# rubendhz/houdini-gsplat-renderer

Hardware: AMD Instinct MI355X
Metric: frames/sec at 1920x1080 + achieved HBM GB/s (blend kernel) (higher is better)
Workload: dtype f32

## Files before the change

houdini-gsplat-renderer_amd/csrc/gsr_api.hip:

```cpp
#include <hip/hip_runtime.h>

#include <cmath>
#include <cstdarg>
#include <cstdio>
#include <cstring>
#include <chrono>
#include <algorithm>
#include <new>
#include <vector>

#include "../../include/gsplat_hip.h"
#include "gsr_device.h"
#include "k_binning.h"
#include "k_blend.h"
#include "k_cluster.h"
#include "k_colour.h"
#include "k_preprocess.h"
#ifdef GSR_HOST_TIMING
static double g_t_verdict = 0, g_acc_py = 0, g_acc_pre = 0, g_acc_launch = 0; static long g_acc_n = 0;
static double now_us() { return std::chrono::duration<double, std::micro>(std::chrono::steady_clock::now().time_since_epoch()).count(); }
#endif
#include "k_sort.h"
#include "k_wire.h"
#include "gsr_frame_plan.h"
// ... 105 lines not shown
    float* dpyr = nullptr;
    size_t dpyr_cap = 0;
    uint32_t* dactive = nullptr;
    int dpar = 0;
    bool dpyr_built = false;
    bool sorted_dculled = false;
    uint32_t* hist = nullptr;
    size_t hist_cap = 0;
    uint32_t* totals = nullptr;
    uint2* pvA = nullptr;
    size_t pair_cap = 0;
    int32_t *sstart = nullptr, *send = nullptr;
    uint4* tile_work = nullptr;
    size_t tile_cap = 0;
    uint4* tile_work_a = nullptr;
    float* tbuf = nullptr;
    size_t tbuf_cap = 0;
    float* hpyr2 = nullptr;
    uint32_t* slab = nullptr;
    bool slab_dirty = false;
    int32_t* redo = nullptr;
    int32_t* order = nullptr;
    size_t order_cap = 0;
    bool order_valid = false;
    int order_age = 0;
    int order_sig[6] = {0, 0, 0, 0, 0, 0}, order_per_xcd = 0;
    uint32_t* st_scan = nullptr;
    GsrTilePartial* partial = nullptr;
    uint32_t* sup_work = nullptr;
    int sup_par = 0;
// ... 268 lines not shown
    return ok;
}

static void slot_free_splat_arrays(FrameSlot& sl)
{
    dev_free(sl.rec); dev_free(sl.keyA); dev_free(sl.keyB); dev_free(sl.valA); dev_free(sl.valB); dev_free(sl.blk_cnt);
    dev_free(sl.zwin); dev_free(sl.cseg);
    sl.sort_valid = false;
}

static void slot_destroy(FrameSlot& sl)
{
    slot_free_splat_arrays(sl);
    dev_free(sl.hist); dev_free(sl.totals);
    dev_free(sl.pvA);
    dev_free(sl.sstart); dev_free(sl.send); dev_free(sl.tile_work); dev_free(sl.order); dev_free(sl.sup_work); dev_free(sl.fb); dev_free(sl.fb32); dev_free(sl.aovb); dev_free(sl.bgb);
    dev_free(sl.hpyr); dev_free(sl.hpyr_next); dev_free(sl.hraw); dev_free(sl.hstat); dev_free(sl.hpyr2); dev_free(sl.slab); dev_free(sl.tile_work_a); dev_free(sl.tbuf); dev_free(sl.ccnt); dev_free(sl.bkt_key); dev_free(sl.bkt_val); dev_free(sl.bkt_cnt); dev_free(sl.d_counts); dev_free(sl.st_scan); dev_free(sl.partial);
    if (sl.h_end) (void)hipHostFree(sl.h_end); dev_free(sl.depth_stage); dev_free(sl.dpyr); dev_free(sl.dactive);
    dev_free(sl.redo); dev_free(sl.lazy_ctr); dev_free(sl.colour_evals);
    dev_free(sl.counters); dev_free(sl.d_n);
    if (sl.h_total) (void)hipHostFree(sl.h_total);
    if (sl.h_counters) (void)hipHostFree(sl.h_counters);
    dev_free(sl.d_frame);
    if (sl.ev_ok)
        for (int k = 0; k < GSR_STAGE_EVENTS; ++k)
            if (sl.ev[k]) (void)hipEventDestroy(sl.ev[k]);
    if (sl.ev_done) (void)hipEventDestroy(sl.ev_done);
    if (sl.ev_user) (void)hipEventDestroy(sl.ev_user);
    for (int k = 0; k < GSR_HOST_BANDS_MAX; ++k) if (sl.ev_band[k]) (void)hipEventDestroy(sl.ev_band[k]);
    if (sl.ev_pairs) (void)hipEventDestroy(sl.ev_pairs);
    if (sl.own) (void)hipStreamDestroy(sl.own);
// ... 820 lines not shown
    if (j.timing && (j.timing_all || k >= 5)) HIP_TRY(hipEventRecord(sl.ev[k], sl.stream));
    return GSR_OK;
}

static GsrRangeArgs range_args(gsr_context* c, FrameSlot& sl)
{
    const FrameJob& j = sl.job;
    GsrRangeArgs a;
    a.totals = sl.totals; a.n_super = j.n_super; a.sstart = sl.sstart; a.send = sl.send; a.host_total = sl.h_total_dev;
    a.ticket = j.ticket; a.max_pairs = (unsigned long long)GSR_MAX_PAIRS; a.redo_count = reinterpret_cast<uint32_t*>(sl.lazy_ctr);
    a.lazy_hint = c->lazy_hint; a.n_sorted = sl.d_n; a.k1_counts = sl.d_counts; a.sorted_keys = sl.keyA;
    a.depth_active = j.dcull ? sl.dactive + j.dpar : (const uint32_t*)nullptr;
    return a;
}

static int queue_blend(gsr_context* c, FrameSlot& sl, bool with_depth, bool guarded)
{
    const FrameJob& j = sl.job;
    const GsrFrame& f = j.f;
    hipStream_t s = sl.stream;
    if (j.local_tiles > 0) {
        if (!j.direct) HIP_TRY(hipStreamWaitEvent(s, sl.ev_user, 0));
        GsrBlendArgs a;
        a.guard = guarded ? sl.dactive + j.dpar : (const uint32_t*)nullptr; a.guard_want = 0u;
        {
            const bool persp = f.pr[8] == 0.0f && f.pr[9] == 0.0f && f.pr[12] == 0.0f && f.pr[13] == 0.0f && f.pr[14] == -1.0f && f.pr[15] == 0.0f;
            a.near_alpha = persp ? 0.5f * (1.0f - f.pr[10]) : 0.0f;
            a.near_scale = persp ? 1.12f : 0.0f;
        }
        a.tile_cov = (with_depth && j.dcull && !j.dblind) ? sl.dpyr + 4 * sl.dpyr_cap : (const float*)nullptr;
        a.idx_mask = f.idx_mask; a.zq0 = f.zq0; a.zqs = f.zqs;
        a.tile_dmax = (with_depth && j.dcull && !j.dblind && f.idx_mask != 0xffffffffu) ? sl.dpyr + (size_t)(2 * j.dpar) * sl.dpyr_cap + f.pyr_off[0] : (const float*)nullptr;
        a.width = f.width; a.height = f.height; a.tiles_x = f.tiles_x; a.local_tiles = j.local_tiles;
        a.shard = GsrShard{f.shard_index, f.shard_count, f.shard_rpb}; a.band_rows = j.band_rows;
        a.super_shift = f.super_shift; a.rect_shift = f.rect_shift; a.stiles_x = f.stiles_x; a.use_map = j.use_map ? 1 : 0; a.flags = f.flags;
        a.list_cap = (int32_t)std::min<size_t>(sl.pair_cap, (size_t)0x7fffffff);
        a.sup_work = (a.use_map && c->opt_swizzle >= 2 && sl.sup_work) ? sl.sup_work + 256 * sl.sup_par : nullptr;
        a.slab = j.phase; a.tbuf = sl.tbuf; a.tile_work_a = sl.tile_work_a;
// ... 98 lines not shown
        HIP_TRY(hipGetLastError());
    }
    if ((rc = mark(sl, 5))) return rc;
    sl.job.blend_guess_plain = j.d_depth != nullptr && j.dcull && !c->depth_active && !j.deferred && j.f.idx_mask == 0xffffffffu && !j.aov_target && j.bg.kind == 0;
    if ((rc = queue_blend(c, sl, j.d_depth != nullptr && !sl.job.blend_guess_plain, sl.job.blend_guess_plain))) return rc;
    return mark(sl, 6);
}

static int queue_frame_end(gsr_context* c, FrameSlot& sl)
{
    const FrameJob& j = sl.job;
    hipStream_t s = sl.stream;
    GsrSumArgs g;
    g.n_tiles = j.local_tiles; g.tiles_x = j.f.tiles_x; g.tiles_y = j.f.tiles_y; g.shard = GsrShard{j.f.shard_index, j.f.shard_count, j.f.shard_rpb};
    g.super_shift = j.f.super_shift; g.stiles_x = j.f.stiles_x; g.n_super = j.n_super;
    GsrHorizonArgs hz{};
    hz.list_cap = (int32_t)std::min<size_t>(sl.pair_cap, (size_t)0x7fffffff);
    if (c->opt_cull && c->opt_cull != 3 && j.n > 0 && !j.deferred && (c->opt_cull >= 2 || j.cull || j.phase == 2 || (c->cull_pol.vis_unculled >= 300000u && c->cull_pol.holdoff <= 2))) {
        hz.raw = sl.hraw; hz.pyr_in = sl.hpyr; hz.pyr_out = sl.hpyr_next; hz.dilate = j.f.cull_dilate; hz.culled = j.cull ? 1 : 0; hz.lists = sl.pvA; hz.geoA = c->geoA;
        for (int l = 0; l < GSR_PYR_LEVELS; ++l) hz.pyr_off[l] = j.f.pyr_off[l];
        hz.cam[0] = j.f.cam[0]; hz.cam[1] = j.f.cam[1]; hz.cam[2] = j.f.cam[2];
        hz.host_end = j.cull ? sl.h_end_dev : nullptr; hz.ticket = j.ticket;
        hz.stat = sl.hstat;
        hz.stat_in_use = (j.cull && j.dcull && j.dstat) ? 1 : 0;
        hz.depth_culled = (j.dcull && !j.dblind) ? 1 : 0;
        hz.idx_mask = j.f.idx_mask;
        static const bool dbgv = std::getenv("GSR_DEBUG_VIOL") != nullptr;
        if (dbgv) {
            if (!sl.dbg_viol && hipMalloc(reinterpret_cast<void**>(&sl.dbg_viol), 80 * 4) != hipSuccess) sl.dbg_viol = nullptr;
            if (sl.dbg_viol) (void)hipMemsetAsync(sl.dbg_viol, 0, 80 * 4, s);
            hz.dbg = sl.dbg_viol;
        }
    }
    if (j.phase == 2) { hz.slab = 2; hz.tile_work_a = sl.tile_work_a; }
    const int nblocks8 = ((j.f.tiles_x + 7) >> 3) * ((j.f.tiles_y + 7) >> 3);
    hipLaunchKernelGGL(k_tile_pass, dim3((unsigned)nblocks8), dim3(64), 0, s, sl.tile_work, g, sl.sstart, sl.send, hz, sl.partial, sl.st_scan);
    uint32_t* const prefix_arg = (j.f.sh_order > 0 && c->opt_lazy) ? c->prefix : (uint32_t*)nullptr;
    const uint32_t* const redo_arg = j.lazy ? reinterpret_cast<const uint32_t*>(sl.lazy_ctr) : (const uint32_t*)nullptr;
    uint32_t* const work_next = sl.sup_work ? sl.sup_work + 256 * (sl.sup_par ^ 1) : (uint32_t*)nullptr;
    sl.horizon_valid = hz.raw != nullptr;
    sl.hstat_valid = hz.raw != nullptr;
    const int osig[6] = {j.f.width, j.f.height, j.f.shard_index, j.f.shard_count, j.f.shard_rpb, j.f.super_shift};
    const bool order_due = c->opt_swizzle >= 3 || (c->opt_swizzle == 2 && c->order_pays);
    const bool order_kept = !order_due && c->opt_swizzle == 2 && c->opt_order_keep > 0 && sl.order_valid && sl.order_age < c->opt_order_keep &&
                            std::memcmp(osig, sl.order_sig, sizeof osig) == 0;
    const bool order_refresh = !order_due && !order_kept && c->opt_swizzle == 2 && c->opt_order_keep > 0 && c->n >= 1000000u;
    if (order_kept) sl.order_age += 1; else sl.order_valid = false;
    const bool order_now = j.use_map && (order_due || order_refresh) && j.local_tiles > 0 && j.n_super <= 256 && sl.sup_work;
    const int per_xcd = 2 * ((j.n_super + 15) / 16) << (2 * j.f.super_shift);
    if (order_now) {
        const size_t want = (size_t)8 * per_xcd;
        if (want > sl.order_cap) {
            HIP_TRY(hipStreamSynchronize(s));
            dev_free(sl.order);
            sl.order_cap = 0;
            int rc = dev_alloc(&sl.order, want);
            if (rc) return rc;
            sl.order_cap = want;
        }
    }
    const bool fused_order = order_now && c->opt_fuse_order != 0;
    if (sl.horizon_valid) sl.hpyr_re = std::min(c->cull_pol.dilate, GSR_DILATE_EXACT_MAX);
    if (fused_order) {
        const GsrOrderArgs oa{sl.tile_work, j.f.tiles_y, sl.sup_work + 256 * sl.sup_par, per_xcd, sl.order};
        const int ndil = sl.horizon_valid ? nblocks8 : 0;
        hipLaunchKernelGGL(k_frame_end_order, dim3(9u + (unsigned)((ndil + TO_THREADS / 64 - 1) / (TO_THREADS / 64))), dim3(TO_THREADS), 0, s, sl.partial, nblocks8, ndil, g, sl.counters, sl.d_n, sl.d_frame,
                           prefix_arg, redo_arg, sl.colour_evals, sl.lazy_ctr + 1, sl.sstart, sl.send, c->lazy_hint, work_next, hz, sl.st_scan, sl.hpyr_re, oa);
        HIP_TRY(hipGetLastError());
    } else if (sl.horizon_valid) {
        hipLaunchKernelGGL(k_frame_end, dim3((unsigned)nblocks8 + 1u), dim3(SW_THREADS), 0, s, sl.partial, nblocks8, g, sl.counters, sl.d_n, sl.d_frame,
                           prefix_arg, redo_arg, sl.colour_evals, sl.lazy_ctr + 1, sl.sstart, sl.send, c->lazy_hint, work_next, hz, sl.st_scan, sl.hpyr_re);
        HIP_TRY(hipGetLastError());
    } else {
        hipLaunchKernelGGL(k_sum_work, dim3(1), dim3(SW_THREADS), 0, s, sl.partial, nblocks8, g, sl.counters, sl.d_n, sl.d_frame,
                           prefix_arg, redo_arg, sl.colour_evals, sl.lazy_ctr + 1, sl.sstart, sl.send, c->lazy_hint, work_next, hz, sl.st_scan);
        HIP_TRY(hipGetLastError());
    }
    if (sl.horizon_valid) {
        std::swap(sl.hpyr, sl.hpyr_next);
        const int sig[7] = {j.f.width, j.f.height, j.f.shard_index, j.f.shard_count, j.f.shard_rpb, j.f.super_shift, (int)c->geo_gen};
        std::memcpy(sl.horizon_sig, sig, sizeof sig);
        sl.horizon_cam = j.args.cam;
    }
    if (order_now) {
        if (!fused_order) {
            hipLaunchKernelGGL(k_tile_order, dim3(8), dim3(TO_THREADS), 0, s, sl.tile_work, g, j.f.tiles_y, sl.sup_work + 256 * sl.sup_par,
                               per_xcd, sl.order);
            HIP_TRY(hipGetLastError());
        }
        std::memcpy(sl.order_sig, osig, sizeof osig);
// ... 115 lines not shown
template <typename T>
static int regrow(hipStream_t s, T*& p, size_t& cap, size_t count, size_t new_cap)
{
    HIP_TRY(hipStreamSynchronize(s));
    dev_free(p);
    cap = 0;
    const int rc = dev_alloc(&p, count);
    if (rc) return rc;
    cap = new_cap;
    return GSR_OK;
}

static int abandon_attempt(FrameSlot& sl, bool redo)
{
    if (sl.sup_work) (void)hipMemsetAsync(sl.sup_work + 256 * sl.sup_par, 0, 256 * sizeof(uint32_t), sl.stream);
    sl.sort_valid = false;
    sl.job.redo = redo;
    sl.job.open = false;
    return GSR_OK;
}

static int render_again(gsr_context* c, const FrameArgs& a, int phase, FrameSlot** used)
{
    c->frame_no -= 1;
    c->st.frames -= 1;
    FrameSlot* sl = nullptr;
    int rc = frame_begin(c, a, &sl, false, phase);
    if (rc) return rc;
    if ((rc = frame_finish(c, *sl))) return rc;
    if (used) *used = sl;
// ... 51 lines not shown
    if (o.grow) {
        const size_t floor_ = sl.pvA ? 0 : std::min<size_t>((size_t)2 * j.n + 4096, (size_t)1 << 22);
        const size_t want = std::max<size_t>((size_t)D + D / 4 + 4096, std::max(floor_, c->pair_want));
        const int rc = regrow(sl.stream, sl.pvA, sl.pair_cap, want + 4, want);
        if (rc) return frame_abort(sl, rc);
        c->pair_want = std::max(c->pair_want, want);
    }
    if (o.end == GSR_FE_SLAB_OVERRUN) {
        c->st.frames_requeued += 1;
        return abandon_attempt(sl, true);
    }
    if (o.back_end == GSR_BE_TRUNCATED) c->st.frames_truncated += 1;
    if (o.back_end == GSR_BE_REQUEUED) {
        c->st.frames_requeued += 1;
        if (sl.sup_work) (void)hipMemsetAsync(sl.sup_work + 256 * sl.sup_par, 0, 256 * sizeof(uint32_t), sl.stream);
    }
    if (o.back_end == GSR_BE_QUEUED || o.back_end == GSR_BE_REQUEUED) {
        const int rc = queue_back_end(c, sl);
        if (rc) return frame_abort(sl, rc);
    }
    sl.last_pairs = D;
    if (o.guard_miss) {
        j.blend_guess_plain = false;
        const int rc = queue_blend(c, sl, true, false);
        if (rc) return frame_abort(sl, rc);
    }
    if (o.end == GSR_FE_PHASE_2) {
        const int rc = queue_slab_mid(c, sl);
        if (rc) return frame_abort(sl, rc);
        if (j.timing) { sl.ev_pending = true; sl.ev_all = false; }
// ... 120 lines not shown
    j.dcull = p.dcull; j.local_sort = p.local || p.local_phase; j.bn_items = p.bn_items; j.bn_grid = p.bn_grid; j.k1_grid = p.k1_grid;
    j.f.cull_dilate = p.cull_dilate;
    j.f.phase = p.phase;
    c->st.frames_jumped += p.jumped;
    c->st.frames_culled += p.cull;
    c->st.frames_slab += p.phase == 1;
    c->st.frames_lazy += p.lazy && n > 0 && phase_in == 0;
    j.ticket = ++sl.ticket ? sl.ticket : ++sl.ticket;
    if (j.timing) harvest_slot(c, sl);

    j.direct = sl.stream == c->stream;
    if (!j.direct) HIP_TRY(hipEventRecord(sl.ev_user, c->stream));

    if ((size_t)j.local_tiles + 1 > sl.tile_cap || !sl.sstart) {
        HIP_TRY(hipStreamSynchronize(s));
        dev_free(sl.tile_work); dev_free(sl.tile_work_a); dev_free(sl.sstart); dev_free(sl.send); dev_free(sl.redo);
        sl.tile_cap = 0;
        if ((rc = dev_alloc(&sl.tile_work, (size_t)j.local_tiles + 1)) || (rc = dev_alloc(&sl.tile_work_a, (size_t)j.local_tiles + 1)) || (rc = dev_alloc(&sl.sstart, (size_t)65536 + 1)) ||
            (rc = dev_alloc(&sl.send, (size_t)65536 + 1)) || (rc = dev_alloc(&sl.redo, (size_t)j.local_tiles + 1))) return rc;
        sl.tile_cap = (size_t)j.local_tiles + 1;
    }
    if (j.phase == 1 && j.out_px > sl.tbuf_cap && (rc = regrow(s, sl.tbuf, sl.tbuf_cap, j.out_px, j.out_px))) return rc;
    if (j.use_map && (rc = build_tile_map(c, f))) return rc;
    j.d_depth = a.depth;
    if (a.depth && !a.depth_is_device) {
        const size_t npx = (size_t)cam->width * cam->height;
        if (npx > sl.depth_cap && (rc = regrow(s, sl.depth_stage, sl.depth_cap, npx, npx))) return rc;
        HIP_TRY(hipMemcpyAsync(sl.depth_stage, a.depth, npx * 4, hipMemcpyHostToDevice, s));
        j.d_depth = sl.depth_stage;
    }
    if (a.bg.kind != 0) {
        j.bg.kind = a.bg.kind; j.bg.format = a.bg.format;
        std::memcpy(j.bg.rgba, a.bg.rgba, sizeof j.bg.rgba);
// ... 820 lines not shown
```

houdini-gsplat-renderer_amd/csrc/gsr_device.h:

```cpp
#pragma once
#ifdef GSR_KPROF
#include <hip/hip_runtime.h>
__device__ unsigned long long g_kprof[8][16];
__device__ unsigned int g_kprof_blk[5][2][8192];
#define KPROF_BLK_BEGIN const unsigned long long kp0_ = wall_clock64();
#define KPROF_BLK_END(k, items) { if (threadIdx.x == 0 && blockIdx.x < 8192) { g_kprof_blk[k][0][blockIdx.x] = (unsigned int)(wall_clock64() - kp0_); g_kprof_blk[k][1][blockIdx.x] = (unsigned int)(items); } }
#define KPROF(k, i) { if (blockIdx.x == 0 && threadIdx.x == 0) g_kprof[k][i] = wall_clock64(); }
#define KPROFB(k, i, blk) { if (blockIdx.x == (blk) && threadIdx.x == 0) g_kprof[k][i] = wall_clock64(); }
#else
#define KPROF(k, i)
#define KPROFB(k, i, blk)
#define KPROF_BLK_BEGIN
#define KPROF_BLK_END(k, items)
#endif

#include <hip/hip_runtime.h>
#include <stdint.h>
#include "gsr_mailbox.h"

#define GSR_TILE_PX 16
#define GSR_WAVE 64

struct __attribute__((aligned(16))) GsrRecord {
    float cx, cy, hx, hy;
// ... 33 lines not shown
    int32_t rect_shift;
    int32_t phase;
    uint32_t idx_mask;
    float zq0, zqs;
};
#define GSR_ZQ_SHIFT 23
#define GSR_ZQ_MAX 511.0f
#define GSR_SLAB_BINS 1024
#define GSR_FLAG_NO_ALPHA_RADIUS 1
#define GSR_FLAG_NO_SAT          2
#define GSR_FLAG_FULL_KEYS       4
#define GSR_FLAG_LAZY_NO_PREFIX  8
#define GSR_FLAG_CULL_ROUNDS    16
#define GSR_FLAG_NO_DEPTH_CLASS 32
#define GSR_FLAG_NO_ZCODES      64

#ifndef BK_BUCKETS
#define BK_BUCKETS 1024
#endif
#ifndef BK_CAP
#define BK_CAP 8192
#endif
#define BK_STRIDE 64

__device__ __forceinline__ float gsr_fma(float a, float b, float c) { return __builtin_fmaf(a, b, c); }

__device__ __forceinline__ uint32_t gsr_zq(float zw, float z0, float zs)
{
    const float t = __builtin_fminf(__builtin_fmaxf((zw - z0) * zs, 0.0f), GSR_ZQ_MAX);
    return (uint32_t)t;
// ... 185 lines not shown
```

houdini-gsplat-renderer_amd/csrc/k_blend.h:

```cpp
#pragma once
#include <type_traits>
#include "gsr_device.h"
#include "k_preprocess.h"
#include "k_cluster.h"

#ifndef BL_ROUND
#define BL_ROUND 64
#endif
#ifndef BL_WAVES_PER_EU
#define BL_WAVES_PER_EU 6
#endif
#ifndef BL_CHECK
#define BL_CHECK 4
#endif
#ifndef BL_BATCH
#define BL_BATCH 256
#endif
#ifndef BL_CHECK_AOVD
#define BL_CHECK_AOVD 2
#endif
#define BL_QCAP 2048
#define BL_PAIR_F4_MAX 6
#define GSR_T_MIN 6.103515625e-05f

#ifdef BL_PROFILE
#define BLP_MAX_WG 65536
__device__ unsigned long long g_blend_prof[BLP_MAX_WG][4][16];
#define BLP(i) { const long long now_ = clock64(); prof[i] += (unsigned long long)(now_ - tlast); tlast = now_; }
#else
#define BLP(i)
#endif

__device__ __forceinline__ uint32_t gsr_tile_weight(const uint4& w) { return w.z * 32u + w.y * 8u + (w.x >> 1); }

#ifdef GSR_DEBUG_XCC
__device__ uint32_t g_dbg_xcc[4];
#endif
struct GsrBlendArgs {
    int32_t width, height;
    int32_t tiles_x;
    int32_t local_tiles;
    GsrShard shard;
    int32_t band_rows;
    int32_t super_shift;
    int32_t rect_shift;
    int32_t stiles_x;
    int32_t use_map;
    int32_t flags;
    int32_t list_cap;
    uint32_t* sup_work;
    int32_t slab;
    float* tbuf;
    const uint4* tile_work_a;
    const uint32_t* guard;
    uint32_t guard_want;
    float near_alpha, near_scale;
    const float* tile_cov;
    uint32_t idx_mask;
    float zq0, zqs;
    const float* tile_dmax;
    int32_t row_lo, row_hi;
    int32_t out_format;
    void* out_packed;
};

#if BL_WAVES_PER_EU > 0
#define BL_OCC __attribute__((amdgpu_waves_per_eu(BL_WAVES_PER_EU)))
#else
#define BL_OCC
#endif
struct GsrLazyArgs {
    GsrFrame f;
    const uint4* colrow;
    int32_t* redo;
    uint32_t* redo_count;
};
struct GsrBgArgs {
    int32_t kind;
    int32_t format;
    float rgba[4];
    const void* image;
};
template <bool HAS_DEPTH, bool LAZY, bool AOV = false, bool OVER = false>
__device__ __forceinline__ void
gsr_blend_tile(const GsrBlendArgs& a, const int32_t* __restrict__ tile_map, const uint2* __restrict__ svals,
               const int32_t* __restrict__ sstart, const int32_t* __restrict__ send,
               const GsrRecord* __restrict__ recs, float4* __restrict__ out, uint4* __restrict__ tile_work,
               const float* __restrict__ zwin, const float* __restrict__ depth, const GsrLazyArgs& lz, float2* __restrict__ aov = nullptr,
               const GsrBgArgs* __restrict__ bg = nullptr)
{
    constexpr bool ZSTAGE = HAS_DEPTH || AOV;
    constexpr int PF4 = 5;
    __shared__ float4 slist[4][(BL_ROUND / 2) * PF4];
    __shared__ float2 szl[ZSTAGE ? 4 : 1][ZSTAGE ? BL_ROUND / 2 : 1];
    __shared__ uint32_t q[BL_QCAP];
    __shared__ __attribute__((aligned(16))) uint32_t scnt[2][4];
    __shared__ uint32_t sdone[2][4];
// ... 49 lines not shown

    const int st = (gty >> a.super_shift) * a.stiles_x + (tx >> a.super_shift);
    const int s = sstart[st];
    const int e_ = send[st] < a.list_cap ? send[st] : a.list_cap;
    const int n = e_ > s ? e_ - s : 0;
    if (!HAS_DEPTH && a.guard && (guard_now != 0u) != (a.guard_want != 0u)) return;

    gsr_v2f C01 = {0.0f, 0.0f};
    float C2 = 0.0f, T = 1.0f;
    float Z = 0.0f;
    bool wave_done = false;
    if (a.slab == 2) {
        const uint4 wa = a.tile_work_a[tile];
        if (wa.w & 1u) {
            if (tid == 0) tile_work[tile] = make_uint4(0u, 0u, 0u, 1u | 0x8000u | (0xffffu << 16));
            return;
        }
        if (pix_ok) {
            const size_t at = (size_t)(lty * GSR_TILE_PX + (wave >> 1) * 8 + (lane >> 3)) * a.width + (size_t)(tx * GSR_TILE_PX + (wave & 1) * 8 + (lane & 7));
            const float4 c = out[at];
            C01 = (gsr_v2f){c.x, c.y}; C2 = c.z; T = a.tbuf[at];
            if constexpr (AOV) Z = aov[at].x;
        }
        wave_done = __all(!pix_ok || T < GSR_T_MIN);
    }
    bool u_done = false;
    uint32_t my_last_u = 0;
    uint32_t es_u = 0xffu;
    bool u_all = false;
    uint32_t fetched = 0;
// ... 322 lines not shown
        for (int i = 0; i < 9; ++i) o[i] = prof[i];
        o[9] = 1ull; o[10] = (unsigned long long)round; o[11] = wall0; o[12] = wall_clock64();
        o[13] = occ_lanes; o[14] = occ_evals; o[15] = occ_half | (occ_none << 32);
    }
#endif
    __syncthreads();
    if (lane == 0) { atomicAdd(&sevals, my_evals); if (HAS_DEPTH && d_met) sdmet = 1u; }
    __syncthreads();
    if (HAS_DEPTH && !d_init) init_depth();
    const uint32_t es_c = ext_steps_of(max(max(slast[0], slast[1]), max(slast[2], slast[3])));
    if (!HAS_DEPTH) { u_all = saturated; es_u = es_c; }
    else if (!u_all) {
        const uint32_t dl = sdone[(round - 1) & 1][0] & sdone[(round - 1) & 1][1] & sdone[(round - 1) & 1][2] & sdone[(round - 1) & 1][3];
        if (round > 0 ? (dl & 2u) != 0u : __syncthreads_and(u_done ? 1 : 0) != 0) { u_all = true; es_u = round > 0 ? ext_steps_of(max(max(slastu[0], slastu[1]), max(slastu[2], slastu[3]))) : 0u; }
    }
    if (tid == 0) {
        const int rd = scan_pos + 1024;
        const uint32_t fs = (uint32_t)(first_hit_step < 0 ? 0 : (first_hit_step > 0x1fff ? 0x1fff : first_hit_step)) | (sdmet ? 0x2000u : 0u);
        const uint4 tw = make_uint4((uint32_t)(rd < n ? rd : n), fetched, sevals, (saturated ? 1u : 0u) | (fs << 1) | (u_all ? 0x8000u : 0u) | (es_c << 16) | (es_u << 24));
        tile_work[tile] = tw;
        if (a.sup_work && gsr_tile_weight(tw)) atomicAdd(&a.sup_work[st], gsr_tile_weight(tw));
    }
}

template <bool HAS_DEPTH>
__global__ void __launch_bounds__(256) BL_OCC
k_blend(GsrBlendArgs a, const int32_t* __restrict__ tile_map, const uint2* __restrict__ svals,
        const int32_t* __restrict__ sstart, const int32_t* __restrict__ send,
        const GsrRecord* __restrict__ recs, float4* __restrict__ out, uint4* __restrict__ tile_work,
        const float* __restrict__ zwin, const float* __restrict__ depth, GsrLazyArgs lz)
{
    gsr_blend_tile<HAS_DEPTH, false>(a, tile_map, svals, sstart, send, recs, out, tile_work, zwin, depth, lz);
}
template <bool HAS_DEPTH>
__global__ void __launch_bounds__(256)
k_blend_lazy(GsrBlendArgs a, const int32_t* __restrict__ tile_map, const uint2* __restrict__ svals,
             const int32_t* __restrict__ sstart, const int32_t* __restrict__ send,
// ... 253 lines not shown
        if (own) h = !opaque ? __builtin_inff() : (c2 ? hnew : slab_d2 * 1.05f);
        if (inside) hz.raw[gty * g.tiles_x + tx] = (own && !(opaque && (w.w & 0x4000u) == 0u)) ? -h : h;
    }
}

__device__ __forceinline__ void
gsr_sum_work(const GsrTilePartial* __restrict__ partial, int nblocks, GsrSumArgs g, unsigned long long* __restrict__ counters,
           const uint32_t* __restrict__ n_visible, unsigned long long* __restrict__ summary ,
           uint32_t* __restrict__ prefix ,
           const uint32_t* __restrict__ redo_count ,
           uint32_t* __restrict__ colour_evals ,
           unsigned long long* __restrict__ colour_total ,
           const int32_t* __restrict__ sstart, const int32_t* __restrict__ send,
           uint32_t* __restrict__ lazy_hint ,
           uint32_t* __restrict__ sup_work_next ,
           GsrHorizonArgs hz, uint32_t* __restrict__ st_scan )
{
    SWP(0)
    __shared__ unsigned long long s_sum[3];
    __shared__ uint32_t s_unsat, s_est, s_cev, s_wmax, s_nfin, s_nused, s_viol;
    unsigned long long old2 = 0, old4 = 0, old5 = 0, old_ct = 0;
    uint32_t nvis = 0, nredo = 0, my_cev = 0, my_m = 0;
    int my_s0 = 0, my_e0 = 0;
    if (threadIdx.x == 0) {
        old2 = counters[2]; old4 = counters[4]; old5 = counters[5];
        nvis = *n_visible;
        nredo = redo_count ? *redo_count : 0u;
        if (colour_evals) old_ct = *colour_total;
        s_unsat = 0; s_est = 0; s_cev = 0; s_wmax = 0; s_nfin = 0; s_nused = 0; s_viol = 0;
    }
    if (threadIdx.x < 3) s_sum[threadIdx.x] = 0;
    if (colour_evals) my_cev = colour_evals[threadIdx.x];
    if ((int)threadIdx.x < g.n_super) { my_m = st_scan[threadIdx.x]; my_s0 = sstart[threadIdx.x]; my_e0 = send[threadIdx.x]; }
    unsigned long long sc = 0, fe = 0, ev = 0;
    uint32_t wmax = 0, unsat = 0, nused = 0, nfin = 0, viol = 0;
    for (int i = (int)threadIdx.x; i < nblocks; i += SW_THREADS) {
        const GsrTilePartial p = partial[i];
        sc += p.scanned; fe += p.fetched; ev += p.evals; unsat += p.unsat; nused += p.nused; nfin += p.nfin; viol |= p.viol;
        wmax = p.wmax > wmax ? p.wmax : wmax;
    }
    __syncthreads();
#pragma unroll
    for (int d = 32; d > 0; d >>= 1) {
        sc += __shfl_down(sc, d, 64); fe += __shfl_down(fe, d, 64); ev += __shfl_down(ev, d, 64); unsat += __shfl_down(unsat, d, 64);
        nused += __shfl_down(nused, d, 64); nfin += __shfl_down(nfin, d, 64);
        { const uint32_t o = __shfl_down(wmax, d, 64); wmax = o > wmax ? o : wmax; }
    }
    const bool any_viol = __ballot(viol != 0u) != 0ull;
    if ((threadIdx.x & 63) == 0) {
        atomicAdd(&s_sum[0], sc); atomicAdd(&s_sum[1], fe); atomicAdd(&s_sum[2], ev); atomicAdd(&s_unsat, unsat); atomicMax(&s_wmax, wmax);
// ... 35 lines not shown
                                    ((hz.culled || ((unsigned long long)s_nfin * 10ull >= (unsigned long long)s_nused * 3ull && s_nused > 0u)) ? GSR_HINT_CULL_PAYS : 0u);
        const unsigned long long t2 = old2 + s_sum[1], t4 = old4 + s_sum[0], t5 = old5 + s_sum[2];
        counters[1] = s_sum[1]; counters[2] = t2; counters[3] = s_sum[0]; counters[4] = t4; counters[5] = t5;
        if (colour_evals) *colour_total = old_ct + s_cev;
        summary[0] = 0ull; summary[1] = s_sum[1]; summary[2] = t2; summary[3] = s_sum[0]; summary[4] = t4; summary[5] = t5;
        summary[6] = (unsigned long long)nvis;
        summary[7] = (unsigned long long)nredo;
    }
    SWP(5)
}
__global__ void __launch_bounds__(SW_THREADS)
k_sum_work(const GsrTilePartial* __restrict__ partial, int nblocks, GsrSumArgs g, unsigned long long* __restrict__ counters,
           const uint32_t* __restrict__ n_visible, unsigned long long* __restrict__ summary, uint32_t* __restrict__ prefix,
           const uint32_t* __restrict__ redo_count, uint32_t* __restrict__ colour_evals, unsigned long long* __restrict__ colour_total,
           const int32_t* __restrict__ sstart, const int32_t* __restrict__ send, uint32_t* __restrict__ lazy_hint,
           uint32_t* __restrict__ sup_work_next, GsrHorizonArgs hz, uint32_t* __restrict__ st_scan)
{
    gsr_sum_work(partial, nblocks, g, counters, n_visible, summary, prefix, redo_count, colour_evals, colour_total, sstart, send, lazy_hint,
                 sup_work_next, hz, st_scan);
}

__device__ __forceinline__ void
gsr_horizon_dilate(const float* __restrict__ raw, int tiles_x, int tiles_y, int r, const GsrHorizonArgs& hz, float* __restrict__ pyr, const int b,
                   const int lane )
{
    const int lx = (lane & 1) | ((lane >> 1) & 2) | ((lane >> 2) & 4), ly = ((lane >> 1) & 1) | ((lane >> 2) & 2) | ((lane >> 3) & 4);
    const int nbx = (tiles_x + 7) >> 3;
    const int by = b / nbx, bx = b - by * nbx;
    const int tx = bx * 8 + lx, ty = by * 8 + ly;
    const bool inside = tx < tiles_x && ty < tiles_y;
    float v = 0.0f;
    if (inside) {
        const int x0 = max(tx - r, 0), x1 = min(tx + r, tiles_x - 1), y0 = max(ty - r, 0), y1 = min(ty + r, tiles_y - 1);
        bool allc = true;
// ... 16 lines not shown
        atomicMax(reinterpret_cast<uint32_t*>(pyr) + hz.pyr_off[4] + (by >> 1) * gsr_pyr_dim(tiles_x, 4) + (bx >> 1), __float_as_uint(v));
        atomicMax(reinterpret_cast<uint32_t*>(pyr) + hz.pyr_off[5] + (by >> 2) * gsr_pyr_dim(tiles_x, 5) + (bx >> 2), __float_as_uint(v));
    }
}
__global__ void __launch_bounds__(64)
k_horizon_dilate(const float* __restrict__ raw, int tiles_x, int tiles_y, int r, GsrHorizonArgs hz, float* __restrict__ pyr)
{
    gsr_horizon_dilate(raw, tiles_x, tiles_y, r, hz, pyr, (int)blockIdx.x, (int)threadIdx.x);
}

__global__ void __launch_bounds__(SW_THREADS)
k_frame_end(const GsrTilePartial* __restrict__ partial, int nblocks, GsrSumArgs g, unsigned long long* __restrict__ counters,
            const uint32_t* __restrict__ n_visible, unsigned long long* __restrict__ summary, uint32_t* __restrict__ prefix,
            const uint32_t* __restrict__ redo_count, uint32_t* __restrict__ colour_evals, unsigned long long* __restrict__ colour_total,
            const int32_t* __restrict__ sstart, const int32_t* __restrict__ send, uint32_t* __restrict__ lazy_hint,
            uint32_t* __restrict__ sup_work_next, GsrHorizonArgs hz, uint32_t* __restrict__ st_scan, int dilate_r)
{
    if ((int)blockIdx.x == nblocks) {
        gsr_sum_work(partial, nblocks, g, counters, n_visible, summary, prefix, redo_count, colour_evals, colour_total, sstart, send, lazy_hint,
                     sup_work_next, hz, st_scan);
        return;
    }
    if (threadIdx.x >= 64) return;
    gsr_horizon_dilate(hz.raw, g.tiles_x, g.tiles_y, dilate_r, hz, hz.pyr_out, (int)blockIdx.x, (int)threadIdx.x);
}

#define TO_THREADS 1024
#define TO_LEVELS 128
__device__ __forceinline__ void
gsr_tile_order(const uint4* __restrict__ tile_work, const GsrSumArgs& g, int tiles_y, const uint32_t* __restrict__ sup_work, int cap,
               int32_t* __restrict__ order, const int xcd)
{
    __shared__ uint32_t s_sup[256];
    __shared__ uint32_t s_own[64];
    __shared__ uint32_t s_hist[TO_LEVELS];
// ... 84 lines not shown
}
__global__ void __launch_bounds__(TO_THREADS)
k_tile_order(const uint4* __restrict__ tile_work, GsrSumArgs g, int tiles_y, const uint32_t* __restrict__ sup_work, int cap,
             int32_t* __restrict__ order)
{
    gsr_tile_order(tile_work, g, tiles_y, sup_work, cap, order, (int)blockIdx.x);
}

struct GsrOrderArgs { const uint4* tile_work; int32_t tiles_y; const uint32_t* sup_work; int32_t cap; int32_t* order; };
__global__ void __launch_bounds__(TO_THREADS)
k_frame_end_order(const GsrTilePartial* __restrict__ partial, int nblocks, int ndilate , GsrSumArgs g,
                  unsigned long long* __restrict__ counters, const uint32_t* __restrict__ n_visible, unsigned long long* __restrict__ summary,
                  uint32_t* __restrict__ prefix, const uint32_t* __restrict__ redo_count, uint32_t* __restrict__ colour_evals,
                  unsigned long long* __restrict__ colour_total, const int32_t* __restrict__ sstart, const int32_t* __restrict__ send,
                  uint32_t* __restrict__ lazy_hint, uint32_t* __restrict__ sup_work_next, GsrHorizonArgs hz, uint32_t* __restrict__ st_scan, int dilate_r,
                  GsrOrderArgs oa)
{
    const int b = (int)blockIdx.x;
    if (b < 8) {
        gsr_tile_order(oa.tile_work, g, oa.tiles_y, oa.sup_work, oa.cap, oa.order, b);
        return;
    }
    if (b == 8) {
        if (threadIdx.x >= SW_THREADS) return;
        gsr_sum_work(partial, nblocks, g, counters, n_visible, summary, prefix, redo_count, colour_evals, colour_total, sstart, send, lazy_hint,
                     sup_work_next, hz, st_scan);
        return;
    }
    static_assert(TO_THREADS % 64 == 0 && SW_THREADS % 64 == 0, "early exits are by whole wavefronts");
    const int blk = (b - 9) * (TO_THREADS / 64) + (int)(threadIdx.x >> 6);
    if (blk >= ndilate) return;
    gsr_horizon_dilate(hz.raw, g.tiles_x, g.tiles_y, dilate_r, hz, hz.pyr_out, blk, (int)(threadIdx.x & 63u));
}
```

Measured before the change: 4433.

## Fold tile-pass horizon/stat work into blend kernel epilogue

Moves the per-tile post-processing that k_tile_pass did (horizon raw depth, supertile scan maxima, flag bits) into an epilogue of each blend tile, writing compact per-tile flags. The summing kernel then reduces tile_work plus flags directly instead of per-block partials, and k_tile_pass is launched only when a new opt-in flag is set. This removes a kernel launch and a re-read of tile work and lists, at the cost of extra registers and latency inside the blend kernel, plus new memsets for st_scan and hraw state.

After: 4315. 0.974x the previous value.

```diff
diff --git a/houdini-gsplat-renderer_amd/csrc/gsr_api.hip b/houdini-gsplat-renderer_amd/csrc/gsr_api.hip
--- a/houdini-gsplat-renderer_amd/csrc/gsr_api.hip
+++ b/houdini-gsplat-renderer_amd/csrc/gsr_api.hip
@@ -143,6 +143,8 @@
     uint4* tile_work = nullptr;
     size_t tile_cap = 0;
     uint4* tile_work_a = nullptr;
+    uint32_t* tile_flags = nullptr;
+    int hraw_sig[5] = {0, 0, 0, 0, 0};
     float* tbuf = nullptr;
     size_t tbuf_cap = 0;
     float* hpyr2 = nullptr;
@@ -441,7 +443,7 @@
     slot_free_splat_arrays(sl);
     dev_free(sl.hist); dev_free(sl.totals);
     dev_free(sl.pvA);
-    dev_free(sl.sstart); dev_free(sl.send); dev_free(sl.tile_work); dev_free(sl.order); dev_free(sl.sup_work); dev_free(sl.fb); dev_free(sl.fb32); dev_free(sl.aovb); dev_free(sl.bgb);
+    dev_free(sl.sstart); dev_free(sl.send); dev_free(sl.tile_work); dev_free(sl.tile_flags); dev_free(sl.order); dev_free(sl.sup_work); dev_free(sl.fb); dev_free(sl.fb32); dev_free(sl.aovb); dev_free(sl.bgb);
     dev_free(sl.hpyr); dev_free(sl.hpyr_next); dev_free(sl.hraw); dev_free(sl.hstat); dev_free(sl.hpyr2); dev_free(sl.slab); dev_free(sl.tile_work_a); dev_free(sl.tbuf); dev_free(sl.ccnt); dev_free(sl.bkt_key); dev_free(sl.bkt_val); dev_free(sl.bkt_cnt); dev_free(sl.d_counts); dev_free(sl.st_scan); dev_free(sl.partial);
     if (sl.h_end) (void)hipHostFree(sl.h_end); dev_free(sl.depth_stage); dev_free(sl.dpyr); dev_free(sl.dactive);
     dev_free(sl.redo); dev_free(sl.lazy_ctr); dev_free(sl.colour_evals);
@@ -1292,14 +1294,58 @@
     return a;
 }
 
+static GsrHorizonArgs horizon_args(gsr_context* c, FrameSlot& sl, bool for_blend)
+{
+    const FrameJob& j = sl.job;
+    const bool tile_pass = (j.f.flags & GSR_FLAG_TILE_PASS) != 0;
+    GsrHorizonArgs hz{};
+    hz.list_cap = (int32_t)std::min<size_t>(sl.pair_cap, (size_t)0x7fffffff);
+    if (c->opt_cull && c->opt_cull != 3 && j.n > 0 && !j.deferred && (for_blend || c->opt_cull >= 2 || j.cull || j.phase == 2 || (c->cull_pol.vis_unculled >= 300000u && c->cull_pol.holdoff <= 2))) {
+        hz.raw = sl.hraw; hz.pyr_in = sl.hpyr; hz.pyr_out = sl.hpyr_next; hz.dilate = j.f.cull_dilate; hz.culled = j.cull ? 1 : 0; hz.lists = sl.pvA; hz.geoA = c->geoA;
+        for (int l = 0; l < GSR_PYR_LEVELS; ++l) hz.pyr_off[l] = j.f.pyr_off[l];
+        hz.cam[0] = j.f.cam[0]; hz.cam[1] = j.f.cam[1]; hz.cam[2] = j.f.cam[2];
+        hz.host_end = j.cull ? sl.h_end_dev : nullptr; hz.ticket = j.ticket;
+        hz.stat = sl.hstat;
+        hz.stat_in_use = (j.cull && j.dcull && j.dstat) ? 1 : 0;
+        hz.depth_culled = (j.dcull && !j.dblind) ? 1 : 0;
+        hz.idx_mask = j.f.idx_mask;
+        static const bool dbgv = std::getenv("GSR_DEBUG_VIOL") != nullptr;
+        if (dbgv && for_blend != tile_pass) {
+            if (!sl.dbg_viol && hipMalloc(reinterpret_cast<void**>(&sl.dbg_viol), 80 * 4) != hipSuccess) sl.dbg_viol = nullptr;
+            if (sl.dbg_viol) (void)hipMemsetAsync(sl.dbg_viol, 0, 80 * 4, sl.stream);
+            hz.dbg = sl.dbg_viol;
+        }
+    }
+    if (j.phase == 2) { hz.slab = 2; hz.tile_work_a = sl.tile_work_a; }
+    return hz;
+}
+
 static int queue_blend(gsr_context* c, FrameSlot& sl, bool with_depth, bool guarded)
 {
     const FrameJob& j = sl.job;
     const GsrFrame& f = j.f;
     hipStream_t s = sl.stream;
+    const bool tile_end = j.phase != 1 && !(f.flags & GSR_FLAG_TILE_PASS);
+    const GsrHorizonArgs hz = tile_end ? horizon_args(c, sl, true) : GsrHorizonArgs{};
+    const int hsig[5] = {f.tiles_x, f.tiles_y, f.shard_index, f.shard_count, f.shard_rpb};
+    if (f.shard_count > 1 && sl.hraw && std::memcmp(hsig, sl.hraw_sig, sizeof hsig) != 0) {
+        HIP_TRY(hipMemsetAsync(sl.hraw, 0, (size_t)f.tiles_x * f.tiles_y * sizeof(float), s));
+        std::memcpy(sl.hraw_sig, hsig, sizeof hsig);
+    }
+    if (hz.raw && j.local_tiles == 0)
+        HIP_TRY(hipMemsetAsync(hz.pyr_out + hz.pyr_off[4], 0, sizeof(float) * (size_t)(gsr_pyr_dim(f.tiles_x, 4) * gsr_pyr_dim(f.tiles_y, 4) + gsr_pyr_dim(f.tiles_x, 5) * gsr_pyr_dim(f.tiles_y, 5)), s));
     if (j.local_tiles > 0) {
         if (!j.direct) HIP_TRY(hipStreamWaitEvent(s, sl.ev_user, 0));
         GsrBlendArgs a;
+        a.te = GsrTileEndArgs{};
+        if (tile_end) {
+            GsrTileEndArgs& te = a.te;
+            te.flags = sl.tile_flags; te.st_scan = sl.st_scan; te.tiles_y = f.tiles_y;
+            te.raw = hz.raw; te.pyr_in = hz.pyr_in; te.pyr_out = hz.pyr_out; te.culled = hz.culled; te.dilate = hz.dilate; te.geoA = hz.geoA;
+            for (int l = 0; l < GSR_PYR_LEVELS; ++l) te.pyr_off[l] = hz.pyr_off[l];
+            te.cam[0] = hz.cam[0]; te.cam[1] = hz.cam[1]; te.cam[2] = hz.cam[2];
+            te.stat = hz.stat; te.stat_in_use = hz.stat_in_use; te.depth_culled = hz.depth_culled; te.dbg = hz.dbg;
+        }
         a.guard = guarded ? sl.dactive + j.dpar : (const uint32_t*)nullptr; a.guard_want = 0u;
         {
             const bool persp = f.pr[8] == 0.0f && f.pr[9] == 0.0f && f.pr[12] == 0.0f && f.pr[13] == 0.0f && f.pr[14] == -1.0f && f.pr[15] == 0.0f;
@@ -1428,27 +1474,11 @@
     GsrSumArgs g;
     g.n_tiles = j.local_tiles; g.tiles_x = j.f.tiles_x; g.tiles_y = j.f.tiles_y; g.shard = GsrShard{j.f.shard_index, j.f.shard_count, j.f.shard_rpb};
     g.super_shift = j.f.super_shift; g.stiles_x = j.f.stiles_x; g.n_super = j.n_super;
-    GsrHorizonArgs hz{};
-    hz.list_cap = (int32_t)std::min<size_t>(sl.pair_cap, (size_t)0x7fffffff);
-    if (c->opt_cull && c->opt_cull != 3 && j.n > 0 && !j.deferred && (c->opt_cull >= 2 || j.cull || j.phase == 2 || (c->cull_pol.vis_unculled >= 300000u && c->cull_pol.holdoff <= 2))) {
-        hz.raw = sl.hraw; hz.pyr_in = sl.hpyr; hz.pyr_out = sl.hpyr_next; hz.dilate = j.f.cull_dilate; hz.culled = j.cull ? 1 : 0; hz.lists = sl.pvA; hz.geoA = c->geoA;
-        for (int l = 0; l < GSR_PYR_LEVELS; ++l) hz.pyr_off[l] = j.f.pyr_off[l];
-        hz.cam[0] = j.f.cam[0]; hz.cam[1] = j.f.cam[1]; hz.cam[2] = j.f.cam[2];
-        hz.host_end = j.cull ? sl.h_end_dev : nullptr; hz.ticket = j.ticket;
-        hz.stat = sl.hstat;
-        hz.stat_in_use = (j.cull && j.dcull && j.dstat) ? 1 : 0;
-        hz.depth_culled = (j.dcull && !j.dblind) ? 1 : 0;
-        hz.idx_mask = j.f.idx_mask;
-        static const bool dbgv = std::getenv("GSR_DEBUG_VIOL") != nullptr;
-        if (dbgv) {
-            if (!sl.dbg_viol && hipMalloc(reinterpret_cast<void**>(&sl.dbg_viol), 80 * 4) != hipSuccess) sl.dbg_viol = nullptr;
-            if (sl.dbg_viol) (void)hipMemsetAsync(sl.dbg_viol, 0, 80 * 4, s);
-            hz.dbg = sl.dbg_viol;
-        }
-    }
-    if (j.phase == 2) { hz.slab = 2; hz.tile_work_a = sl.tile_work_a; }
+    const bool tile_pass = (j.f.flags & GSR_FLAG_TILE_PASS) != 0;
+    const GsrHorizonArgs hz = horizon_args(c, sl, false);
     const int nblocks8 = ((j.f.tiles_x + 7) >> 3) * ((j.f.tiles_y + 7) >> 3);
-    hipLaunchKernelGGL(k_tile_pass, dim3((unsigned)nblocks8), dim3(64), 0, s, sl.tile_work, g, sl.sstart, sl.send, hz, sl.partial, sl.st_scan);
+    if (tile_pass) hipLaunchKernelGGL(k_tile_pass, dim3((unsigned)nblocks8), dim3(64), 0, s, sl.tile_work, g, sl.sstart, sl.send, hz, sl.partial, sl.st_scan);
+    const uint32_t* const flags_arg = tile_pass ? (const uint32_t*)nullptr : sl.tile_flags;
     uint32_t* const prefix_arg = (j.f.sh_order > 0 && c->opt_lazy) ? c->prefix : (uint32_t*)nullptr;
     const uint32_t* const redo_arg = j.lazy ? reinterpret_cast<const uint32_t*>(sl.lazy_ctr) : (const uint32_t*)nullptr;
     uint32_t* const work_next = sl.sup_work ? sl.sup_work + 256 * (sl.sup_par ^ 1) : (uint32_t*)nullptr;
@@ -1479,15 +1509,15 @@
         const GsrOrderArgs oa{sl.tile_work, j.f.tiles_y, sl.sup_work + 256 * sl.sup_par, per_xcd, sl.order};
         const int ndil = sl.horizon_valid ? nblocks8 : 0;
         hipLaunchKernelGGL(k_frame_end_order, dim3(9u + (unsigned)((ndil + TO_THREADS / 64 - 1) / (TO_THREADS / 64))), dim3(TO_THREADS), 0, s, sl.partial, nblocks8, ndil, g, sl.counters, sl.d_n, sl.d_frame,
-                           prefix_arg, redo_arg, sl.colour_evals, sl.lazy_ctr + 1, sl.sstart, sl.send, c->lazy_hint, work_next, hz, sl.st_scan, sl.hpyr_re, oa);
+                           prefix_arg, redo_arg, sl.colour_evals, sl.lazy_ctr + 1, sl.sstart, sl.send, c->lazy_hint, work_next, hz, sl.st_scan, sl.hpyr_re, oa, flags_arg);
         HIP_TRY(hipGetLastError());
     } else if (sl.horizon_valid) {
         hipLaunchKernelGGL(k_frame_end, dim3((unsigned)nblocks8 + 1u), dim3(SW_THREADS), 0, s, sl.partial, nblocks8, g, sl.counters, sl.d_n, sl.d_frame,
-                           prefix_arg, redo_arg, sl.colour_evals, sl.lazy_ctr + 1, sl.sstart, sl.send, c->lazy_hint, work_next, hz, sl.st_scan, sl.hpyr_re);
+                           prefix_arg, redo_arg, sl.colour_evals, sl.lazy_ctr + 1, sl.sstart, sl.send, c->lazy_hint, work_next, hz, sl.st_scan, sl.hpyr_re, sl.tile_work, flags_arg);
         HIP_TRY(hipGetLastError());
     } else {
         hipLaunchKernelGGL(k_sum_work, dim3(1), dim3(SW_THREADS), 0, s, sl.partial, nblocks8, g, sl.counters, sl.d_n, sl.d_frame,
-                           prefix_arg, redo_arg, sl.colour_evals, sl.lazy_ctr + 1, sl.sstart, sl.send, c->lazy_hint, work_next, hz, sl.st_scan);
+                           prefix_arg, redo_arg, sl.colour_evals, sl.lazy_ctr + 1, sl.sstart, sl.send, c->lazy_hint, work_next, hz, sl.st_scan, sl.tile_work, flags_arg);
         HIP_TRY(hipGetLastError());
     }
     if (sl.horizon_valid) {
@@ -1633,6 +1663,7 @@
 static int abandon_attempt(FrameSlot& sl, bool redo)
 {
     if (sl.sup_work) (void)hipMemsetAsync(sl.sup_work + 256 * sl.sup_par, 0, 256 * sizeof(uint32_t), sl.stream);
+    if (sl.st_scan) (void)hipMemsetAsync(sl.st_scan, 0, 512 * sizeof(uint32_t), sl.stream);
     sl.sort_valid = false;
     sl.job.redo = redo;
     sl.job.open = false;
@@ -1714,6 +1745,7 @@
     if (o.back_end == GSR_BE_REQUEUED) {
         c->st.frames_requeued += 1;
         if (sl.sup_work) (void)hipMemsetAsync(sl.sup_work + 256 * sl.sup_par, 0, 256 * sizeof(uint32_t), sl.stream);
+        if (sl.st_scan) (void)hipMemsetAsync(sl.st_scan, 0, 512 * sizeof(uint32_t), sl.stream);
     }
     if (o.back_end == GSR_BE_QUEUED || o.back_end == GSR_BE_REQUEUED) {
         const int rc = queue_back_end(c, sl);
@@ -1864,9 +1896,9 @@
 
     if ((size_t)j.local_tiles + 1 > sl.tile_cap || !sl.sstart) {
         HIP_TRY(hipStreamSynchronize(s));
-        dev_free(sl.tile_work); dev_free(sl.tile_work_a); dev_free(sl.sstart); dev_free(sl.send); dev_free(sl.redo);
+        dev_free(sl.tile_work); dev_free(sl.tile_work_a); dev_free(sl.tile_flags); dev_free(sl.sstart); dev_free(sl.send); dev_free(sl.redo);
         sl.tile_cap = 0;
-        if ((rc = dev_alloc(&sl.tile_work, (size_t)j.local_tiles + 1)) || (rc = dev_alloc(&sl.tile_work_a, (size_t)j.local_tiles + 1)) || (rc = dev_alloc(&sl.sstart, (size_t)65536 + 1)) ||
+        if ((rc = dev_alloc(&sl.tile_work, (size_t)j.local_tiles + 1)) || (rc = dev_alloc(&sl.tile_flags, (size_t)j.local_tiles + 1)) || (rc = dev_alloc(&sl.tile_work_a, (size_t)j.local_tiles + 1)) || (rc = dev_alloc(&sl.sstart, (size_t)65536 + 1)) ||
             (rc = dev_alloc(&sl.send, (size_t)65536 + 1)) || (rc = dev_alloc(&sl.redo, (size_t)j.local_tiles + 1))) return rc;
         sl.tile_cap = (size_t)j.local_tiles + 1;
     }
diff --git a/houdini-gsplat-renderer_amd/csrc/gsr_device.h b/houdini-gsplat-renderer_amd/csrc/gsr_device.h
--- a/houdini-gsplat-renderer_amd/csrc/gsr_device.h
+++ b/houdini-gsplat-renderer_amd/csrc/gsr_device.h
@@ -71,6 +71,7 @@
 #define GSR_FLAG_CULL_ROUNDS    16
 #define GSR_FLAG_NO_DEPTH_CLASS 32
 #define GSR_FLAG_NO_ZCODES      64
+#define GSR_FLAG_TILE_PASS     128
 
 #ifndef BK_BUCKETS
 #define BK_BUCKETS 1024
diff --git a/houdini-gsplat-renderer_amd/csrc/k_blend.h b/houdini-gsplat-renderer_amd/csrc/k_blend.h
--- a/houdini-gsplat-renderer_amd/csrc/k_blend.h
+++ b/houdini-gsplat-renderer_amd/csrc/k_blend.h
@@ -36,6 +36,25 @@
 #ifdef GSR_DEBUG_XCC
 __device__ uint32_t g_dbg_xcc[4];
 #endif
+#define GSR_TE_UNSAT 1u
+#define GSR_TE_USED  2u
+#define GSR_TE_FIN   4u
+#define GSR_TE_VIOL  8u
+struct GsrTileEndArgs {
+    uint32_t* flags;
+    uint32_t* st_scan;
+    float* raw;
+    const float* pyr_in;
+    float* pyr_out;
+    int32_t pyr_off[GSR_PYR_LEVELS];
+    int32_t tiles_y;
+    int32_t culled, dilate;
+    const float4* geoA;
+    float cam[3];
+    const float* stat;
+    int32_t stat_in_use, depth_culled;
+    uint32_t* dbg;
+};
 struct GsrBlendArgs {
     int32_t width, height;
     int32_t tiles_x;
@@ -62,6 +81,7 @@
     int32_t row_lo, row_hi;
     int32_t out_format;
     void* out_packed;
+    GsrTileEndArgs te;
 };
 
 #if BL_WAVES_PER_EU > 0
@@ -81,6 +101,80 @@
     float rgba[4];
     const void* image;
 };
+__device__ __forceinline__ void
+gsr_tile_end(const GsrBlendArgs& a, const uint2* __restrict__ lists, const int tile, const int tx, const int gty, const int st,
+             const int s0, const uint32_t len, const uint4 w, const bool a_done)
+{
+    const GsrTileEndArgs& te = a.te;
+    int lane = (int)threadIdx.x;
+    asm volatile("" : "+v"(lane));
+    lane &= 63;
+    if (te.raw && tile == 0) {
+        const int n45 = gsr_pyr_dim(a.tiles_x, 4) * gsr_pyr_dim(te.tiles_y, 4) + gsr_pyr_dim(a.tiles_x, 5) * gsr_pyr_dim(te.tiles_y, 5);
+#pragma unroll 1
+        for (int i = lane; i < n45; i += 64) te.pyr_out[te.pyr_off[4] + i] = 0.0f;
+    }
+    uint4 wa = make_uint4(0u, 0u, 0u, 0u);
+    if (a.slab == 2) wa = a.tile_work_a[tile];
+    float hold = __builtin_inff();
+    if (te.raw && te.culled)
+        hold = gsr_pyr_max(te.pyr_in, te.pyr_off, a.tiles_x, max(tx - te.dilate, 0), max(gty - te.dilate, 0),
+                           min(tx + te.dilate, a.tiles_x - 1), min(gty + te.dilate, te.tiles_y - 1));
+    const uint32_t es_all = (w.w >> 16) & 0xffu;
+    const uint32_t rd_all = (es_all == 0xffu || (es_all << 10) > w.x) ? w.x : (es_all << 10);
+    const bool opaque_all = (w.w & 1u) != 0u;
+    const bool classic_now = opaque_all && (w.w & 0x4000u) == 0u;
+    const bool pred_classic = !(te.stat && te.stat_in_use) || te.stat[gty * a.tiles_x + tx] != 0.0f;
+    const uint32_t es_u = w.w >> 24;
+    const uint32_t rd_u = (es_u == 0xffu || (es_u << 10) > w.x) ? w.x : (es_u << 10);
+    const uint32_t rdc = pred_classic ? rd_all : rd_u;
+    const bool opaque_c = pred_classic ? opaque_all : (classic_now || (w.w & 0x8000u) != 0u);
+    const uint32_t rd = classic_now ? rd_all : rd_u;
+    const bool opaque = classic_now || (w.w & 0x8000u) != 0u;
+    const uint32_t first = ((w.w >> 1) & 0x1fffu) << 10;
+    const uint32_t want = rd + ((rd > first ? rd - first : 0u) >> 2) + 1024u;
+    if (lane == 0 && st < 256) {
+        if (opaque_all && rd_all) atomicMax(&te.st_scan[st], rd_all);
+        if (!opaque_all && !a_done) te.st_scan[256 + st] = 1u;
+    }
+    uint32_t viol = 0u;
+    if (te.raw) {
+        const bool ok = opaque && rd > 0u && rd <= len;
+        const bool c1 = opaque_c && rdc > 0u && rdc <= len && hold < 3.0e38f, c2 = ok && want < len;
+        const bool c3 = ok && !c2 && !(hold < 3.0e38f) && te.depth_culled != 0;
+        const uint32_t i1 = c1 ? lists[(uint32_t)s0 + rdc - 1u].x & a.idx_mask : 0u;
+        const uint32_t i2 = c2 ? lists[(uint32_t)s0 + want].x & a.idx_mask : 0u;
+        const float4 P1 = te.geoA[c1 ? i1 : 0u], P2 = te.geoA[c2 ? i2 : 0u];
+        float klast, hnew;
+        { const float dx = P1.x - te.cam[0], dy = P1.y - te.cam[1], dz = P1.z - te.cam[2]; klast = gsr_fma(dz, dz, gsr_fma(dy, dy, dx * dx)); }
+        { const float dx = P2.x - te.cam[0], dy = P2.y - te.cam[1], dz = P2.z - te.cam[2]; hnew = gsr_fma(dz, dz, gsr_fma(dy, dy, dx * dx)); }
+        const bool none_c = opaque_c && !pred_classic && rdc == 0u;
+        const bool none = opaque && !classic_now && rd == 0u;
+        if (hold < 3.0e38f && !none_c && (!opaque_c || !c1 || !(klast <= hold))) viol = 1u;
+        if (viol && te.dbg && lane == 0) {
+            const uint32_t k = atomicAdd(te.dbg, 1u);
+            if (k < 8u) {
+                uint32_t* o = te.dbg + 1 + 8 * k;
+                o[0] = (uint32_t)tx; o[1] = (uint32_t)gty; o[2] = w.w; o[3] = w.x; o[4] = __float_as_uint(hold); o[5] = __float_as_uint(klast);
+                o[6] = (pred_classic ? 1u : 0u) | (opaque_c ? 2u : 0u) | (c1 ? 4u : 0u) | (classic_now ? 8u : 0u); o[7] = rdc;
+            }
+        }
+        float h = __builtin_inff();
+        if (none) h = 0.0f;
+        else if (opaque) {
+            if (c2) h = hnew;
+            else if (hold < 3.0e38f) h = hold * 1.05f;
+            else if (c3) h = hnew * 1.05f;
+        }
+        if (!a_done && lane == 0) te.raw[gty * a.tiles_x + tx] = !classic_now ? -h : h;
+    }
+    uint32_t fl = viol ? GSR_TE_VIOL : 0u;
+    if (len > 0u) { fl |= GSR_TE_USED; if (opaque && rd > 0u && rd <= len && (unsigned long long)want * 10ull <= (unsigned long long)len * 7ull) fl |= GSR_TE_FIN; }
+    if (a_done) fl |= GSR_TE_USED | GSR_TE_FIN;
+    if (!a_done && !(w.w & 1u) && (w.y || wa.y)) fl |= GSR_TE_UNSAT;
+    if (lane == 0) te.flags[tile] = fl;
+}
+
 template <bool HAS_DEPTH, bool LAZY, bool AOV = false, bool OVER = false>
 __device__ __forceinline__ void
 gsr_blend_tile(const GsrBlendArgs& a, const int32_t* __restrict__ tile_map, const uint2* __restrict__ svals,
@@ -160,6 +254,8 @@
         const uint4 wa = a.tile_work_a[tile];
         if (wa.w & 1u) {
             if (tid == 0) tile_work[tile] = make_uint4(0u, 0u, 0u, 1u | 0x8000u | (0xffffu << 16));
+            if (a.te.flags && __builtin_amdgcn_readfirstlane(tid) < 64)
+                gsr_tile_end(a, svals, tile, tx, gty, st, s, (uint32_t)n, make_uint4(0u, 0u, 0u, 0u), true);
             return;
         }
         if (pix_ok) {
@@ -512,13 +608,16 @@
         const uint32_t dl = sdone[(round - 1) & 1][0] & sdone[(round - 1) & 1][1] & sdone[(round - 1) & 1][2] & sdone[(round - 1) & 1][3];
         if (round > 0 ? (dl & 2u) != 0u : __syncthreads_and(u_done ? 1 : 0) != 0) { u_all = true; es_u = round > 0 ? ext_steps_of(max(max(slastu[0], slastu[1]), max(slastu[2], slastu[3]))) : 0u; }
     }
+    const int rd = scan_pos + 1024;
+    const uint32_t tw_w = (saturated ? 1u : 0u) | (((uint32_t)(first_hit_step < 0 ? 0 : (first_hit_step > 0x1fff ? 0x1fff : first_hit_step)) | (sdmet ? 0x2000u : 0u)) << 1) |
+                          (u_all ? 0x8000u : 0u) | (es_c << 16) | (es_u << 24);
+    const uint4 tw = make_uint4((uint32_t)(rd < n ? rd : n), fetched, sevals, tw_w);
     if (tid == 0) {
-        const int rd = scan_pos + 1024;
-        const uint32_t fs = (uint32_t)(first_hit_step < 0 ? 0 : (first_hit_step > 0x1fff ? 0x1fff : first_hit_step)) | (sdmet ? 0x2000u : 0u);
-        const uint4 tw = make_uint4((uint32_t)(rd < n ? rd : n), fetched, sevals, (saturated ? 1u : 0u) | (fs << 1) | (u_all ? 0x8000u : 0u) | (es_c << 16) | (es_u << 24));
         tile_work[tile] = tw;
         if (a.sup_work && gsr_tile_weight(tw)) atomicAdd(&a.sup_work[st], gsr_tile_weight(tw));
     }
+    if (a.te.flags && __builtin_amdgcn_readfirstlane(tid) < 64)
+        gsr_tile_end(a, svals, tile, tx, gsr_shard_global_row(a.shard, lty), st, s, (uint32_t)n, tw, false);
 }
 
 template <bool HAS_DEPTH>
@@ -802,7 +901,8 @@
            const int32_t* __restrict__ sstart, const int32_t* __restrict__ send,
            uint32_t* __restrict__ lazy_hint ,
            uint32_t* __restrict__ sup_work_next ,
-           GsrHorizonArgs hz, uint32_t* __restrict__ st_scan )
+           GsrHorizonArgs hz, uint32_t* __restrict__ st_scan ,
+           const uint4* __restrict__ tile_work, const uint32_t* __restrict__ tile_flags )
 {
     SWP(0)
     __shared__ unsigned long long s_sum[3];
@@ -822,6 +922,21 @@
     if ((int)threadIdx.x < g.n_super) { my_m = st_scan[threadIdx.x]; my_s0 = sstart[threadIdx.x]; my_e0 = send[threadIdx.x]; }
     unsigned long long sc = 0, fe = 0, ev = 0;
     uint32_t wmax = 0, unsat = 0, nused = 0, nfin = 0, viol = 0;
+    if (tile_flags) {
+        const bool slab2 = hz.slab == 2;
+#pragma unroll 4
+        for (int i = (int)threadIdx.x; i < g.n_tiles; i += SW_THREADS) {
+            uint4 w = tile_work[i];
+            const uint32_t fl = tile_flags[i];
+            uint4 wa = make_uint4(0u, 0u, 0u, 0u);
+            if (slab2) wa = hz.tile_work_a[i];
+            if (wa.w & 1u) w = make_uint4(0u, 0u, 0u, 0u);
+            sc += (unsigned long long)w.x + wa.x; fe += (unsigned long long)w.y + wa.y; ev += (unsigned long long)w.z + wa.z;
+            const uint32_t wt = gsr_tile_weight(w) + gsr_tile_weight(wa);
+            wmax = wt > wmax ? wt : wmax;
+            unsat += (fl & GSR_TE_UNSAT) ? 1u : 0u; nused += (fl & GSR_TE_USED) ? 1u : 0u; nfin += (fl & GSR_TE_FIN) ? 1u : 0u; viol |= fl & GSR_TE_VIOL;
+        }
+    } else
     for (int i = (int)threadIdx.x; i < nblocks; i += SW_THREADS) {
         const GsrTilePartial p = partial[i];
         sc += p.scanned; fe += p.fetched; ev += p.evals; unsat += p.unsat; nused += p.nused; nfin += p.nfin; viol |= p.viol;
@@ -887,10 +1002,11 @@
            const uint32_t* __restrict__ n_visible, unsigned long long* __restrict__ summary, uint32_t* __restrict__ prefix,
            const uint32_t* __restrict__ redo_count, uint32_t* __restrict__ colour_evals, unsigned long long* __restrict__ colour_total,
            const int32_t* __restrict__ sstart, const int32_t* __restrict__ send, uint32_t* __restrict__ lazy_hint,
-           uint32_t* __restrict__ sup_work_next, GsrHorizonArgs hz, uint32_t* __restrict__ st_scan)
+           uint32_t* __restrict__ sup_work_next, GsrHorizonArgs hz, uint32_t* __restrict__ st_scan,
+           const uint4* __restrict__ tile_work, const uint32_t* __restrict__ tile_flags)
 {
     gsr_sum_work(partial, nblocks, g, counters, n_visible, summary, prefix, redo_count, colour_evals, colour_total, sstart, send, lazy_hint,
-                 sup_work_next, hz, st_scan);
+                 sup_work_next, hz, st_scan, tile_work, tile_flags);
 }
 
 __device__ __forceinline__ void
@@ -937,11 +1053,12 @@
             const uint32_t* __restrict__ n_visible, unsigned long long* __restrict__ summary, uint32_t* __restrict__ prefix,
             const uint32_t* __restrict__ redo_count, uint32_t* __restrict__ colour_evals, unsigned long long* __restrict__ colour_total,
             const int32_t* __restrict__ sstart, const int32_t* __restrict__ send, uint32_t* __restrict__ lazy_hint,
-            uint32_t* __restrict__ sup_work_next, GsrHorizonArgs hz, uint32_t* __restrict__ st_scan, int dilate_r)
+            uint32_t* __restrict__ sup_work_next, GsrHorizonArgs hz, uint32_t* __restrict__ st_scan, int dilate_r,
+            const uint4* __restrict__ tile_work, const uint32_t* __restrict__ tile_flags)
 {
     if ((int)blockIdx.x == nblocks) {
         gsr_sum_work(partial, nblocks, g, counters, n_visible, summary, prefix, redo_count, colour_evals, colour_total, sstart, send, lazy_hint,
-                     sup_work_next, hz, st_scan);
+                     sup_work_next, hz, st_scan, tile_work, tile_flags);
         return;
     }
     if (threadIdx.x >= 64) return;
@@ -1056,7 +1173,7 @@
                   uint32_t* __restrict__ prefix, const uint32_t* __restrict__ redo_count, uint32_t* __restrict__ colour_evals,
                   unsigned long long* __restrict__ colour_total, const int32_t* __restrict__ sstart, const int32_t* __restrict__ send,
                   uint32_t* __restrict__ lazy_hint, uint32_t* __restrict__ sup_work_next, GsrHorizonArgs hz, uint32_t* __restrict__ st_scan, int dilate_r,
-                  GsrOrderArgs oa)
+                  GsrOrderArgs oa, const uint32_t* __restrict__ tile_flags)
 {
     const int b = (int)blockIdx.x;
     if (b < 8) {
@@ -1066,7 +1183,7 @@
     if (b == 8) {
         if (threadIdx.x >= SW_THREADS) return;
         gsr_sum_work(partial, nblocks, g, counters, n_visible, summary, prefix, redo_count, colour_evals, colour_total, sstart, send, lazy_hint,
-                     sup_work_next, hz, st_scan);
+                     sup_work_next, hz, st_scan, oa.tile_work, tile_flags);
         return;
     }
     static_assert(TO_THREADS % 64 == 0 && SW_THREADS % 64 == 0, "early exits are by whole wavefronts");
```
